# wei-zeng98/piano-a2s

Hardware: AMD Instinct MI355X
Metric: training clips/sec (12 s, 5-bar) (higher is better)
Workload: dtype f32

## Files before the change

### piano_a2s_amd/csrc/a2s_api.hip

```cpp
#define A2S_SWITCHES_IMPL
#include "a2s_internal.h"

thread_local char a2s_err_msg[512] = {0};
long long a2s_launch_counter = 0;

#define ST ((hipStream_t)stream)

extern "C" {

const char* a2s_last_error(void) { return a2s_err_msg; }
int a2s_version(void) { return 1; }
long long a2s_launch_count(void) { return __atomic_load_n(&a2s_launch_counter, __ATOMIC_RELAXED); }

int a2s_gemm_f32(void* stream, int M, int N, int K, float alpha, const float* A, long sAm, long sAk, const float* B, long sBk,
                 long sBn, float beta, float* C, long ldc, const float* bias, int act, int batch, long bsA, long bsB, long bsC,
                 int splitk, float* workspace, size_t workspace_bytes) {
    return a2s_gemm_impl(ST, M, N, K, alpha, A, sAm, sAk, B, sBk, sBn, beta, C, ldc, bias, act, batch, bsA, bsB, bsC, splitk,
                         workspace, workspace_bytes);
}
int a2s_gemm_f32_affine(void* stream, int M, int N, int K, float alpha, const float* A, long sAm, long sAk, const float* B, long sBk,
                        long sBn, float beta, float* C, long ldc, const float* bias, int act, int batch, long bsA, long bsB, long bsC,
                        int splitk, float* workspace, size_t workspace_bytes, const float* a_scale, const float* a_shift, int a_period,
                        const float* b_scale, const float* b_shift, int b_period) {
    return a2s_gemm_affine_impl(ST, M, N, K, alpha, A, sAm, sAk, B, sBk, sBn, beta, C, ldc, bias, act, batch, bsA, bsB, bsC, splitk,
                                workspace, workspace_bytes, a_scale, a_shift, a_period, b_scale, b_shift, b_period,
                                nullptr, nullptr, nullptr, nullptr, nullptr, nullptr, 0, 0, nullptr, nullptr);
}
int a2s_gemm_f32_affine_scaled(void* stream, int M, int N, int K, float alpha, const float* A, long sAm, long sAk, const float* B, long sBk,
                               long sBn, float beta, float* C, long ldc, const float* bias, int act, int batch, long bsA, long bsB, long bsC,
                               int splitk, float* workspace, size_t workspace_bytes, const float* a_scale, const float* a_shift, int a_period,
                               const float* b_scale, const float* b_shift, int b_period, const float* a_absmax, const float* b_absmax) {
    return a2s_gemm_affine_impl(ST, M, N, K, alpha, A, sAm, sAk, B, sBk, sBn, beta, C, ldc, bias, act, batch, bsA, bsB, bsC, splitk,
                                workspace, workspace_bytes, a_scale, a_shift, a_period, b_scale, b_shift, b_period,
                                nullptr, nullptr, nullptr, nullptr, nullptr, nullptr, 0, 1, a_absmax, b_absmax);
}
int a2s_gemm_f32_bnstats_scaled(void* stream, int M, int N, int K, const float* A, long sAm, long sAk, const float* B, long sBk, long sBn, float* C, long ldc,
                                const float* y, const float* mean, const float* invstd, const float* scale, const float* shift, int period, float* partial,
                                const float* a_absmax, const float* b_absmax) {
    return a2s_gemm_affine_impl(ST, M, N, K, 1.f, A, sAm, sAk, B, sBk, sBn, 0.f, C, ldc, nullptr, 0, 1, 0, 0, 0, 1, nullptr, 0,
                                nullptr, nullptr, 0, nullptr, nullptr, 0, y, mean, invstd, scale, shift, partial, period, 1, a_absmax, b_absmax);
}
int a2s_absmax(void* stream, const float* x, long n, float* out) { return a2s_absmax_impl(ST, x, n, out); }
int a2s_linear_dgrad_bnstats(void* stream, int M, int N, int K, const float* dz, long lda, const float* Wt, float* da, long ldc, const float* y,
                             const float* mean, const float* invstd, const float* scale, const float* shift, int period, float* partial,
                             const float* dz_absmax, const float* w_absmax, float* workspace, size_t workspace_bytes, float* da_absmax_out) {
    return a2s_linear_dgrad_bnstats_impl(ST, M, N, K, dz, lda, Wt, 1, K, da, ldc, y, mean, invstd, scale, shift, period, partial, dz_absmax, w_absmax,
                                         workspace, workspace_bytes, da_absmax_out);
}
size_t a2s_linear_dgrad_ws_bytes(int N, int K) { return a2s_linear_dgrad_ws_bytes_impl(N, K); }
int a2s_linear_fwd(void* stream, int M, int N, int K, const float* y, long lda, const float* W, float* z, long ldc, const float* scale, const float* shift,
                   int period, const float* y_absmax, const float* w_absmax, float* workspace, size_t workspace_bytes) {
    return a2s_linear_fwd_impl(ST, M, N, K, y, lda, W, z, ldc, scale, shift, period, y_absmax, w_absmax, workspace, workspace_bytes);
}
int a2s_linear_wgrad(void* stream, int M, int N, int K, const float* dz, long ldz, const float* y, long lda, float* G, long ldg, const float* scale,
                     const float* shift, int period, const float* dz_absmax, const float* y_absmax, float* workspace, size_t workspace_bytes) {
    return a2s_linear_wgrad_impl(ST, M, N, K, dz, ldz, y, lda, G, ldg, scale, shift, period, dz_absmax, y_absmax, workspace, workspace_bytes);
}
size_t a2s_linear_wgrad_ws_bytes(int M, int K) { return a2s_linear_wgrad_ws_bytes_impl(M, K); }
int a2s_linear_wgrad_eligible(int M, int N, int K, int period) { return a2s_linear_wgrad_ok(M, N, K, 256, 4, 4, period, nullptr, nullptr, nullptr) ? 1 : 0; }
int a2s_tallk_wgrad(void* stream, int M, int Np, int K, const float* P, long ldp, const float* A, long lda, float* G, long ldg, int transposed, float* bias,
                    const float* p_absmax, const float* a_absmax, float* workspace, size_t workspace_bytes) {
    return a2s_tallk_wgrad_impl(ST, M, Np, K, P, ldp, A, lda, G, ldg, transposed, bias, p_absmax, a_absmax, workspace, workspace_bytes);
}
size_t a2s_tallk_wgrad_ws_bytes(int M, int Np, int K) { return a2s_tallk_wgrad_ws_bytes_impl(M, Np, K); }
int a2s_tallk_wgrad_eligible(int M, int Np, int K, long ldp, long lda, long ldg, int transposed) {
    return a2s_tallk_wgrad_ok(M, Np, K, ldp, lda, ldg, transposed, nullptr, nullptr, nullptr, nullptr) ? 1 : 0;
}
int a2s_linear_fwd_eligible(int M, int N, int K, int period) { return a2s_linear_fwd_ok(M, N, K, 4, 4, period, nullptr, nullptr, nullptr) ? 1 : 0; }
int a2s_linear_dgrad_blocks(int M) { return a2s_linear_dgrad_blocks_impl(M); }
int a2s_linear_dgrad_eligible(int M, int N, int K, int period) {
    return a2s_linear_dgrad_ok(M, N, K, 4, 1, K, 4, period, nullptr, nullptr, nullptr, nullptr) ? 1 : 0;
}
int a2s_gemm_f32_bnstats(void* stream, int M, int N, int K, const float* A, long sAm, long sAk, const float* B, long sBk, long sBn, float* C, long ldc,
                         const float* y, const float* mean, const float* invstd, const float* scale, const float* shift, int period, float* partial) {
    return a2s_gemm_affine_impl(ST, M, N, K, 1.f, A, sAm, sAk, B, sBk, sBn, 0.f, C, ldc, nullptr, 0, 1, 0, 0, 0, 1, nullptr, 0,
                                nullptr, nullptr, 0, nullptr, nullptr, 0, y, mean, invstd, scale, shift, partial, period, 0, nullptr, nullptr);
}
int a2s_gemm_bnstats_blocks(int M, int period) { return a2s_cdiv(M, 128) * a2s_gemm_bnstats_slots(period); }
size_t a2s_gemm_workspace_bytes(int M, int N, int batch, int splitk) { return a2s_gemm_workspace_bytes_impl(M, N, batch, splitk); }
int a2s_gemm_pick_splitk(int M, int N, int K, int batch) { return a2s_gemm_pick_splitk_impl(M, N, K, batch); }
void a2s_gemm_debug_tile(int cfg) { a2s_gemm_debug_tile_impl(cfg); }
size_t a2s_note_step_workspace_floats(int H, int E) { return a2s_note_step_workspace_floats_impl(H, E); }
int a2s_debug_set(const char* key, int value) {
    if (!key) return A2S_ERR_ARG;
    const int id = a2s_switch_find(key);
    if (id >= 0) { a2s_switch_store(id, value); return A2S_OK; }
    if (!strcmp(key, "attn_deferred_fast")) { a2s_attn_deferred_fast = value ? 1 : 0; return A2S_OK; }
    if (!strcmp(key, "tallk_wgrad")) { a2s_tallk_wgrad_on = value ? 1 : 0; return A2S_OK; }
    if (!strcmp(key, "tallk_wgrad_max_splits")) { a2s_tallk_wgrad_max_splits = value > 0 ? value : 0; return A2S_OK; }
    if (!strcmp(key, "conv_rows_stage")) { a2s_conv_rows_stage = value & 3; return A2S_OK; }
    if (!strcmp(key, "gemm_tile")) { a2s_gemm_debug_tile_impl(value); return A2S_OK; }
    snprintf(a2s_err_msg, sizeof(a2s_err_msg), "a2s_debug_set: unknown key %s", key);
    return A2S_ERR_ARG;
}
int a2s_env_check(void) {
    if (const char* e = a2s_switch_env_error()) A2S_FAIL(A2S_ERR_ARG, "%s: expected a decimal number >= 0", e);
    return A2S_OK;
}

int a2s_persist_abort_latch(void* device_word) { a2s_persist_latch_set(device_word); return A2S_OK; }

int a2s_debug_get(const char* key) {
    if (!key) return -1;
    const int id = a2s_switch_find(key);
    if (id == A2S_SW_attn_pair_fused_rows) return a2s_attn_pair_fused_rows();
    if (id >= 0) return a2s_sw((a2s_switch)id);
    if (!strcmp(key, "attn_pair_launches")) return (int)a2s_attn_pair_launches();
    if (!strcmp(key, "attn_pair_bwd_launches")) return (int)a2s_attn_pair_bwd_launches();
    if (!strcmp(key, "attn_deferred_fast")) return a2s_attn_deferred_fast;
    if (!strcmp(key, "tallk_wgrad")) return a2s_tallk_wgrad_on;
    if (!strcmp(key, "tallk_wgrad_max_splits")) return a2s_tallk_wgrad_max_splits;
    if (!strcmp(key, "tallk_wgrad_launches")) return (int)a2s_tallk_wgrad_launches();
    if (!strcmp(key, "attn_dk_ahead_launches")) return (int)a2s_attn_dk_ahead_launches();
    if (!strcmp(key, "attn_denc_launches")) return (int)a2s_attn_denc_launches();
    if (!strcmp(key, "dec_mid_launches")) return a2s_dec_mid_launches();
    if (!strcmp(key, "dec_cmb_launches")) return a2s_dec_cmb_launches();
    if (!strcmp(key, "dec_persist_launches")) return a2s_dec_persist_launches();
    if (!strcmp(key, "gru_persist_fwd_launches")) return (int)a2s_gru_persist_fwd_launches();
    if (!strcmp(key, "gru_persist_bwd_launches")) return (int)a2s_gru_persist_bwd_launches();
    if (!strcmp(key, "gru_step_fwd_launches")) return (int)a2s_gru_step_fwd_launches();
    if (!strcmp(key, "gru_step_bwd_launches")) return (int)a2s_gru_step_bwd_launches();
    if (!strcmp(key, "edit_distance_launches")) return (int)a2s_edit_distance_launches();
    if (!strcmp(key, "conv_rows16_c20_launches")) return (int)a2s_conv_rows16_c20_launches();
    if (!strcmp(key, "conv_rows_stage")) return a2s_conv_rows_stage;
    if (!strcmp(key, "conv_rows_stage_launches")) return (int)a2s_conv_rows_stage_launches();
    if (!strcmp(key, "device_cus")) return a2s_device_geometry().cus;
    if (!strcmp(key, "device_xccs")) return a2s_device_geometry().xccs;
    return -1;
}

int a2s_conv3x3(void* stream, const float* x, const float* w, float* y, const float* in_scale, const float* in_shift,
                float* stat_partial, int B, int T, int F, int Cin, int Cout, int flip, float* workspace) {
    return a2s_conv3x3_impl(ST, x, w, y, in_scale, in_shift, stat_partial, B, T, F, Cin, Cout, flip, workspace, nullptr, nullptr, nullptr, nullptr, nullptr, nullptr,
                            nullptr, nullptr);
}
int a2s_conv3x3_ranged(void* stream, const float* x, const float* w, float* y, const float* in_scale, const float* in_shift, const float* in_absmax,
                       float* stat_partial, float* out_absmax, int B, int T, int F, int Cin, int Cout, float* workspace) {
    return a2s_conv3x3_impl(ST, x, w, y, in_scale, in_shift, stat_partial, B, T, F, Cin, Cout, 0, workspace, nullptr, nullptr, nullptr, nullptr, nullptr, nullptr,
                            in_absmax, out_absmax);
}
int a2s_conv3x3_dgrad_bnstats(void* stream, const float* dy, const float* w, float* g, const float* yl, const float* yl_mean, const float* yl_invstd,
                              const float* yl_scale, const float* yl_shift, float* stat_partial, int B, int T, int F, int Cin, int Cout,
                              float* workspace) {
    if (!yl) { snprintf(a2s_err_msg, sizeof(a2s_err_msg), "conv3x3_dgrad_bnstats: yl is required"); return A2S_ERR_ARG; }
    return a2s_conv3x3_impl(ST, dy, w, g, nullptr, nullptr, stat_partial, B, T, F, Cin, Cout, 1, workspace, yl, yl_mean, yl_invstd, yl_scale, yl_shift, nullptr, nullptr, nullptr);
}
int a2s_conv3x3_dgrad_bnstats_scaled(void* stream, const float* dy, const float* w, float* g, const float* yl, const float* yl_mean, const float* yl_invstd,
                                     const float* yl_scale, const float* yl_shift, float* stat_partial, int B, int T, int F, int Cin, int Cout,
                                     float* workspace, const float* dy_absmax) {
    if (!yl) { snprintf(a2s_err_msg, sizeof(a2s_err_msg), "conv3x3_dgrad_bnstats_scaled: yl is required"); return A2S_ERR_ARG; }
    return a2s_conv3x3_impl(ST, dy, w, g, nullptr, nullptr, stat_partial, B, T, F, Cin, Cout, 1, workspace, yl, yl_mean, yl_invstd, yl_scale, yl_shift, dy_absmax, nullptr, nullptr);
}
int a2s_conv3x3_dgrad_bnstats_ranged(void* stream, const float* dy, const float* w, float* g, const float* yl, const float* yl_mean, const float* yl_invstd,
                                     const float* yl_scale, const float* yl_shift, float* stat_partial, int B, int T, int F, int Cin, int Cout,
                                     float* workspace, const float* dy_absmax, float* g_absmax_out) {
    if (!yl) { snprintf(a2s_err_msg, sizeof(a2s_err_msg), "conv3x3_dgrad_bnstats_ranged: yl is required"); return A2S_ERR_ARG; }
    return a2s_conv3x3_impl(ST, dy, w, g, nullptr, nullptr, stat_partial, B, T, F, Cin, Cout, 1, workspace, yl, yl_mean, yl_invstd, yl_scale, yl_shift, dy_absmax, nullptr, g_absmax_out);
}
int a2s_bn_bwd_from_partial(void* stream, const float* g, const float* x, const float* mean, const float* invstd, const float* scale, const float* shift,
                            float* dgamma, float* dbeta, float* dx, const float* partial, int nblocks, float* c12, long rows, int C, int F) {
    return a2s_bn_bwd_from_partial_impl(ST, g, x, mean, invstd, scale, shift, dgamma, dbeta, dx, partial, nblocks, c12, rows, C, F, nullptr);
}
int a2s_bn_bwd_from_partial_amax(void* stream, const float* g, const float* x, const float* mean, const float* invstd, const float* scale, const float* shift,
                                 float* dgamma, float* dbeta, float* dx, const float* partial, int nblocks, float* c12, long rows, int C, int F,
                                 float* dx_absmax) {
    return a2s_bn_bwd_from_partial_impl(ST, g, x, mean, invstd, scale, shift, dgamma, dbeta, dx, partial, nblocks, c12, rows, C, F, dx_absmax);
}
size_t a2s_conv3x3_workspace_floats(int Cin) { return a2s_conv3x3_workspace_floats_impl(Cin); }
int a2s_conv3x3_stat_blocks(int B, int T, int F, int Cin) { return a2s_conv3x3_stat_blocks_impl(B, T, F, Cin); }
int a2s_bn_finalize(void* stream, const float* partial, int nblocks, int C, double count, const float* gamma, const float* beta,
                    float* running_mean, float* running_var, long long* nbt, float* mean, float* invstd, float* scale,
                    float* shift, float eps, float momentum, int training) {
    return a2s_bn_finalize_impl(ST, partial, nblocks, C, count, gamma, beta, running_mean, running_var, nbt, mean, invstd, scale,
                                shift, eps, momentum, training);
}
int a2s_bn_relu_apply(void* stream, const float* x, float* y, const float* scale, const float* shift, long n, int C, int F) {
    return a2s_bn_relu_apply_impl(ST, x, y, scale, shift, n, C, F);
}
int a2s_linear_fwd_f64(void* stream, int M, int N, int K, const float* x, const float* W, float* z, const float* scale, const float* shift, int period) {
    return a2s_linear_fwd_f64_impl(ST, M, N, K, x, W, z, scale, shift, period);
}
int a2s_col_stats_split(void* stream, const float* x, float* partial, long rows, int C, int rows_per_block) {
    return a2s_col_stats_split_impl(ST, x, partial, rows, C, rows_per_block);
}
int a2s_col_stats(void* stream, const float* x, float* partial, long rows, int C, int rows_per_block) {
    return a2s_col_stats_impl(ST, x, partial, rows, C, rows_per_block);
}
int a2s_bn1d_relu_dropout(void* stream, const float* x, float* y, const float* scale, const float* shift, const uint8_t* keep_mask,
                          float inv_keep, long n, int C) {
    return a2s_bn1d_relu_dropout_impl(ST, x, y, scale, shift, keep_mask, inv_keep, n, C);
}
int a2s_gru_gates_fwd(void* stream, const float* gi, long ldgi, const float* gh, long ldgh, const float* hprev, long ldhp,
                      float* hout, long ldho, float* hout2, long ldho2, float* save, int R, int H) {
    return a2s_gru_gates_fwd_impl(ST, gi, ldgi, gh, ldgh, hprev, ldhp, hout, ldho, hout2, ldho2, save, R, H);
}
int a2s_gru_seq_fwd(void* stream, const float* gi_all, long gi_bstride, long gi_tstride, const float* w_hh, const float* b_hh,
                    float* out, long out_bstride, long out_tstride, float* hbuf, float* gh, float* save, float* hn, int B, int T,
                    int H, int reverse, float* workspace, size_t workspace_bytes) {
    return a2s_gru_seq_fwd_impl(ST, gi_all, gi_bstride, gi_tstride, w_hh, b_hh, out, out_bstride, out_tstride, hbuf, gh, save, hn,
                                B, T, H, reverse, workspace, workspace_bytes);
}
int a2s_attn_step_fwd(void* stream, const float* keys, const float* enc, const float* q, long ldq, const float* v, float* ctx,
                      long ldctx, float* ctx2, long ldctx2, float* attw, int B, int T, int H, const int* n_done, int n_rows_total, float* workspace) {
    return a2s_attn_step_fwd_impl(ST, keys, enc, q, ldq, v, ctx, ldctx, ctx2, ldctx2, attw, B, T, H, n_done, n_rows_total, workspace, nullptr);
}
int a2s_attn_step_fwd_rows(void* stream, const float* keys, const float* enc, const float* q, long ldq, const float* v, float* ctx,
                           long ldctx, float* ctx2, long ldctx2, float* attw, int R, int T, int H, float* workspace, int n_clips,
                           const int* clip_order, const int* clip_rank, const int* row_until, int n_active, int step) {
// ... 351 lines not shown
```

### piano_a2s_amd/csrc/a2s_internal.h

```cpp
#pragma once
#include "a2s_common.h"
#include "../../include/a2s.h"
#include "a2s_switches.h"

static inline int a2s_attn_pair_fused_rows(void) {
    const int cap = a2s_sw(A2S_SW_dec_fused_max_rows), v = a2s_sw(A2S_SW_attn_pair_fused_rows);
    return v < cap ? v : cap;
}
static inline unsigned a2s_persist_dbg(void) {
    return (a2s_sw(A2S_SW_persist_force_agent) ? PERSIST_DBG_FORCE_AGENT : 0u) | (a2s_sw(A2S_SW_persist_inject_abort) ? PERSIST_DBG_INJECT_ABORT : 0u);
}

int a2s_absmax_impl(hipStream_t st, const float* x, long n, float* out);
size_t a2s_gemm_workspace_bytes_impl(int M, int N, int batch, int splitk);
int a2s_gemm_pick_splitk_impl(int M, int N, int K, int batch);
int a2s_gemm_bnstats_slots(int period);
void a2s_gemm_debug_tile_impl(int cfg);
int a2s_gemm_affine_impl(hipStream_t st, int M, int N, int K, float alpha, const float* A, long sAm, long sAk,
    const float* B, long sBk, long sBn, float beta, float* C, long ldc, const float* bias, int act,
    int batch, long bsA, long bsB, long bsC, int splitk, float* ws, size_t ws_bytes,
    const float* a_scale, const float* a_shift, int a_period, const float* b_scale, const float* b_shift, int b_period,
    const float* ep_y, const float* ep_mean, const float* ep_invstd, const float* ep_scale, const float* ep_shift,
    float* ep_partial, int ep_period, int two_term, const float* a_absmax, const float* b_absmax);
int a2s_gemm_impl(hipStream_t st, int M, int N, int K, float alpha, const float* A, long sAm, long sAk,
    const float* B, long sBk, long sBn, float beta, float* C, long ldc, const float* bias, int act,
    int batch, long bsA, long bsB, long bsC, int splitk, float* ws, size_t ws_bytes);

size_t a2s_linear_dgrad_ws_bytes_impl(int N, int K);
int a2s_linear_dgrad_blocks_impl(int M);
bool a2s_linear_dgrad_ok(int M, int N, int K, long lda, long sBk, long sBn, long ldc, int period, const void* A, const void* B, const void* C, const void* y);
int a2s_linear_dgrad_bnstats_impl(hipStream_t st, int M, int N, int K, const float* A, long lda, const float* Wt, long sBk, long sBn, float* C, long ldc,
    const float* ep_y, const float* mean, const float* invstd, const float* scale, const float* shift, int period,
    float* partial, const float* a_absmax, const float* b_absmax, float* ws, size_t ws_bytes, float* c_absmax_out);
bool a2s_linear_fwd_ok(int M, int N, int K, long lda, long ldc, int period, const void* A, const void* W, const void* C);
int a2s_linear_fwd_impl(hipStream_t st, int M, int N, int K, const float* A, long lda, const float* W, float* C, long ldc, const float* a_scale,
    const float* a_shift, int period, const float* a_absmax, const float* w_absmax, float* ws, size_t ws_bytes);
int a2s_linear_fwd_f64_impl(hipStream_t st, int M, int N, int K, const float* x, const float* W, float* z, const float* scale, const float* shift, int period);
size_t a2s_linear_wgrad_ws_bytes_impl(int M, int K);
bool a2s_linear_wgrad_ok(int M, int N, int K, long ldz, long lda, long ldg, int period, const void* dz, const void* A, const void* G);
int a2s_linear_wgrad_impl(hipStream_t st, int M, int N, int K, const float* dz, long ldz, const float* A, long lda, float* G, long ldg, const float* a_scale,
    const float* a_shift, int period, const float* dz_absmax, const float* a_absmax, float* ws, size_t ws_bytes);
extern int a2s_tallk_wgrad_on;
extern int a2s_tallk_wgrad_max_splits;
long a2s_tallk_wgrad_launches(void);
size_t a2s_tallk_wgrad_ws_bytes_impl(int M, int Np, int K);
bool a2s_tallk_wgrad_ok(int M, int Np, int K, long ldp, long lda, long ldg, int transposed, const void* P, const void* A, const void* G, const void* bias);
int a2s_tallk_wgrad_impl(hipStream_t st, int M, int Np, int K, const float* P, long ldp, const float* A, long lda, float* G, long ldg, int transposed,
    float* bias, const float* p_absmax, const float* a_absmax, float* ws, size_t ws_bytes);

#define CV_TR 4
#define CV_FT 32
#define CV_CK 20
#define C4_TRACE_WGS 8
#define C4_TRACE_STAGES 24
int a2s_act_bound_impl(hipStream_t st, const float* scale, const float* shift, const float* absmax, int C, float* out);
size_t a2s_conv3x3_workspace_floats_impl(int Cin);
int a2s_conv3x3_impl(hipStream_t st, const float* x, const float* w, float* y, const float* in_scale,
    const float* in_shift, float* stat_partial, int B, int T, int F, int Cin, int Cout, int flip, float* ws,
    const float* yl, const float* yl_mean, const float* yl_invstd, const float* yl_scale, const float* yl_shift,
    const float* x_absmax, const float* in_absmax, float* out_absmax);
int a2s_conv3x3_stat_blocks_impl(int B, int T, int F, int Cin);

size_t a2s_conv3x3_wgrad_workspace_bytes_impl(int Cin, int Cout);
int a2s_conv3x3_wgrad_impl(hipStream_t st, const float* dy, const float* x, const float* in_scale, const float* in_shift, float* dW,
    float* ws, size_t ws_bytes, int B, int T, int F, int Cin, int Cout, const float* bn_y, const float* bn_mean,
    const float* bn_invstd, const float* bn_scale, const float* bn_shift, const float* bn_c12, float* dy_out,
    const float* dy_absmax, const float* act_absmax);

int a2s_bn_finalize_impl(hipStream_t st, const float* partial, int nblocks, int C, double count, const float* gamma,
    const float* beta, float* running_mean, float* running_var, long long* nbt, float* mean,
    float* invstd, float* scale, float* shift, float eps, float momentum, int training);
int a2s_bn_relu_apply_impl(hipStream_t st, const float* x, float* y, const float* scale, const float* shift, long n, int C, int F);
int a2s_col_stats_impl(hipStream_t st, const float* x, float* partial, long rows, int C, int rows_per_block);
int a2s_col_stats_split_impl(hipStream_t st, const float* x, float* partial, long rows, int C, int rows_per_block);
int a2s_bn1d_relu_dropout_impl(hipStream_t st, const float* x, float* y, const float* scale, const float* shift,
    const uint8_t* mask, float inv_keep, long n, int C);
int a2s_bn_bwd_impl(hipStream_t st, const float* g, const float* x, const float* mean, const float* invstd, const float* scale,
    const float* shift, const uint8_t* mask, float inv_keep, float* dgamma, float* dbeta, float* dx, float* partial,
    float* c12, long rows, int C, int F, float* dx_absmax);
int a2s_bn_bwd_from_partial_impl(hipStream_t st, const float* g, const float* x, const float* mean, const float* invstd, const float* scale,
    const float* shift, float* dgamma, float* dbeta, float* dx, const float* partial, int nblocks, float* c12,
    long rows, int C, int F, float* dx_absmax);
int a2s_bn_bwd_stats_impl(hipStream_t st, const float* g, const float* x, const float* mean, const float* invstd, const float* scale,
    const float* shift, const uint8_t* mask, float inv_keep, float* partial, float* sums, long rows, int C, int F);
int a2s_bn_bwd_apply_impl(hipStream_t st, const float* g, const float* x, const float* mean, const float* invstd, const float* scale,
    const float* shift, const uint8_t* mask, float inv_keep, const float* sums_local, const float* sums_global,
    double count_global, float* dgamma, float* dbeta, float* dx, float* c12, long rows, int C, int F);
int a2s_bn_bwd_sums_from_partial_impl(hipStream_t st, const float* partial, int nblocks, int C, float* sums);
int a2s_bn_bwd_c12_from_sums_impl(hipStream_t st, const float* sums_local, const float* sums_global, double count_global, float* dgamma, float* dbeta,
    float* c12, int C);
size_t a2s_bn_bwd_partial_floats_impl(long rows, int C, int F);
void a2s_absmax_small_launch(hipStream_t st, const float* w, int n, float* out);

int a2s_channel_absmax_impl(hipStream_t st, const float* x, long rows, int C, int F, float* out);
bool a2s_conv_rows_eligible(int F, int Cin);
int a2s_conv_rows_blocks(int B, int T, int F);
size_t a2s_conv_rows_workspace_floats(int Cin);
long a2s_conv_rows16_c20_launches(void);
extern int a2s_conv_rows_stage;
long a2s_conv_rows_stage_launches(void);
int a2s_conv3x3_rows_impl(hipStream_t st, const float* x, const float* w, float* y, const float* in_scale, const float* in_shift,
    const float* in_absmax, float* stat_partial, float* out_absmax, int B, int T, int F, int Cin, int Cout, int flip,
    float* ws, const float* yl, const float* yl_mean, const float* yl_invstd, const float* yl_scale, const float* yl_shift,
    const float* x_absmax);

bool a2s_wgrad_rows_eligible(int F, int Cin, int Cout);
int a2s_conv3x3_wgrad_rows_bn_impl(hipStream_t st, const float* g, const float* y, const float* mean, const float* invstd, const float* scale,
    const float* shift, const float* c12, const float* g_absmax, int g_absmax_n, const float* y_absmax, float* dz_out,
    float* dz_absmax_out, const float* x, const float* in_scale, const float* in_shift, float* dW, float* ws, size_t ws_bytes,
    int B, int T, int F, int Cin, int Cout, const float* act_absmax);
int a2s_conv3x3_wgrad_rows_impl(hipStream_t st, const float* dy, const float* x, const float* in_scale, const float* in_shift, float* dW, float* ws,
    size_t ws_bytes, int B, int T, int F, int Cin, int Cout, const float* dy_absmax, const float* act_absmax);

struct StepFinArgs {
    const float* logits; long ldl;
    float* probs; long probs_bstride;
    const long long* gt; long gt_bstride;
    const float* emb;
    float* xnext; long ldx;
    const uint8_t* drop; float inv_keep;
    int* argmax_out; long am_bstride;
    int* eos_seen; long long* lengths; int* n_done; int* steps_exec;
    const int* t_base;
    const int* row_until;
    int n_clips;
    int R, V, E, t, teacher_force, eos_id, max_t;
};
struct a2s_grammar_ref { const signed char* next; int n_states; int* row_state; };
struct a2s_metre_ref { const int* dur_ticks; const uint8_t* cls; const uint8_t* fillable; int n_fillable; int* row_metre; };
int a2s_gru_gates_fwd_impl(hipStream_t st, const float* gi, long ldgi, const float* gh, long ldgh, const float* hprev,
    long ldhp, float* hout, long ldho, float* hout2, long ldho2, float* save, int R, int H);
int a2s_gru_bptt_step_impl(hipStream_t st, const float* dgh, const float* w_hh_t, const float* dhz_in, const float* dout, long ld_dout,
    const float* save, const float* hprev, long ld_hprev, float* dgi, long ld_dgi, float* dgh_out, float* dgh2,
    long ld_dgh2, float* dhz_out, int R, int H);
int a2s_skinny_gemm_acc_impl(hipStream_t st, const float* A, long lda, const float* Bt, long ldb, float* Cm, long ldc, int R, int N, int K);
long a2s_gru_step_fwd_launches(void);
long a2s_gru_step_bwd_launches(void);
int a2s_gru_seq_fwd_impl(hipStream_t st, const float* gi_all, long gi_bstride, long gi_tstride, const float* w_hh,
    const float* b_hh, float* out, long out_bstride, long out_tstride, float* hbuf, float* gh,
    float* save, float* hn, int B, int T, int H, int reverse, float* ws, size_t ws_bytes);
int a2s_attn_step_fwd_impl(hipStream_t st, const float* Kmat, const float* enc, const float* q, long ldq, const float* v,
    float* ctx, long ldctx, float* ctx2, long ldctx2, float* attw, int B, int T, int H,
    const int* n_done, int n_rows_total, float* ws, const a2s_attn_rows* rows = nullptr, a2s_attn_deferred* defer = nullptr);
int a2s_log_softmax_rows_impl(hipStream_t st, const float* x, long ldx, float* y, long ldy, int* argmax_out, int R, int V);
int a2s_embed_rows_impl(hipStream_t st, const float* table, const long long* ids64, const int* ids32, long id_stride,
    int const_id, float* out, long ldo, int col0, int R, int E, const uint8_t* drop, float inv_keep);
int a2s_note_decoder_fwd_impl(hipStream_t st, const a2s_note_dec_args& a, int* steps_done);
int a2s_note_decoder_fwd_grammar_impl(hipStream_t st, const a2s_note_dec_args& a, const a2s_grammar_ref& g, int* steps_done);
int a2s_note_decoder_fwd_metre_impl(hipStream_t st, const a2s_note_dec_args& a, const a2s_grammar_ref& g, const a2s_metre_ref* mt, int* steps_done);
int a2s_note_decoder_fwd_pair_impl(hipStream_t su, hipStream_t sl, const a2s_note_dec_args& au, const a2s_note_dec_args& al, const int* pair_order,
    const int* pair_rank, const int* pair_n_active, int* done_u, int* done_l);
int a2s_staff_emb_fwd_impl(hipStream_t st, const float* note_emb, const float* const* w ,
    const long long* ids64, const int* ids32, long id_bstride, const long long* lengths,
    long len_stride, float* out, long ldo, int col0, float* hsave, int R, int maxlen, int E, int S);
int a2s_note_decoder_zero_unwritten(hipStream_t st, const a2s_note_dec_args& a, const char* who );
size_t a2s_attn_workspace_floats_impl(int B, int T, int H, int groups);
size_t a2s_attn_bulk_lds(size_t shm, int n_active, int backward);
long a2s_attn_pair_launches(void);
struct AttnPairStep { const int* clip_order; const int* clip_rank; int n_clips; int n_active; int step; int G; int chunk; };
int a2s_pair_events(const char* who, hipEvent_t** ev_out);
static inline int a2s_record_wait(hipEvent_t ev, hipStream_t from, hipStream_t to, const char* who) {
    hipError_t e = hipEventRecord(ev, from);
    if (e == hipSuccess) e = hipStreamWaitEvent(to, ev, 0);
    if (e != hipSuccess) A2S_FAIL(A2S_ERR_HIP, "%s: event: %s", who, hipGetErrorString(e));
    return A2S_OK;
}

int a2s_log_softmax_bwd_rows_impl(hipStream_t st, const float* g, const float* y, long outer_stride, int inner, float* dx,
    int R, int V, int n_outer, int time_major);
int a2s_gru_gates_bwd_impl(hipStream_t st, const float* dh_a, long lda, const float* dh_b, long ldb, const float* save,
    const float* hprev, long ldhp, float* dgi, long ldgi, float* dgh, long ldgh, float* dgh2, long ldgh2,
    float* dhprev, long lddp, int R, int H);
int a2s_attn_step_bwd_impl(hipStream_t st, const float* Kmat, const float* enc, const float* q, long ldq, const float* v,
    const float* attw, const float* ctx, long ldctx, const float* dctx_a, long ldda, const float* dctx_b,
    long lddb, float* dctx_out, long lddo, float* dq, long lddq, float* ds_out, int B, int T, int H, float* ws,
    const a2s_attn_rows* rows = nullptr);
int a2s_attn_dk_accum_impl(hipStream_t st, const float* Kmat, const float* q_all, const float* ds_all, const float* v,
    float* dK, float* dv_partial, int B, int T, int S, int H, const int* row_until, int groups);
int a2s_attn_denc_accum_impl(hipStream_t st, const float* attw_all, const float* dctx_all, float* dEnc, int B, int T, int S, int H2,
    const int* row_until, int groups);
long a2s_attn_dk_ahead_launches(void);
long a2s_attn_denc_launches(void);
int a2s_col_sum_impl(hipStream_t st, const float* x, long ld, float* out, long rows, int C, float alpha, float beta, float* ws, size_t ws_floats);
// ... 227 lines not shown
```

### piano_a2s_amd/csrc/a2s_linear.hip

```cpp
#include "a2s_internal.h"

#define LIN_BM 128
#define LIN_K 256
#define LIN_RS 288
#define LIN_NTH 512
#define LIN_LDS (2 * 2 * LIN_BM * LIN_RS)

typedef unsigned lu32x4 __attribute__((ext_vector_type(4)));

struct LinDgradArgs {
    const float* A; long lda;
    const unsigned char* planes;
    float* C; long ldc;
    const float* ep_y;
    const float* mean; const float* invstd; const float* scale; const float* shift;
    float* partial;
    const float* a_absmax; const float* b_absmax;
    int M, N, period, channels;
    float* c_absmax_out;
};

__global__ __launch_bounds__(256) void lin_pack_planes_k(const float* __restrict__ W, long ld, int N, int K, const float* __restrict__ absmax,
                                                         unsigned char* __restrict__ out) {
    const long id = (long)blockIdx.x * 256 + threadIdx.x;
    const int kgroups = K >> 3, nks = K >> 5;
    const int n = (int)(id / kgroups), kg = (int)(id % kgroups);
    if (n >= N) return;
    const float ps = ldexpf(1.f, pow2_scale_exp(*absmax, 12));
    const f32x4 v0 = *reinterpret_cast<const f32x4*>(W + (long)n * ld + kg * 8);
    const f32x4 v1 = *reinterpret_cast<const f32x4*>(W + (long)n * ld + kg * 8 + 4);
    float x[8];
#pragma unroll
    for (int i = 0; i < 4; ++i) { x[i] = __builtin_amdgcn_fmed3f(v0[i] * ps, -65000.f, 65000.f); x[4 + i] = __builtin_amdgcn_fmed3f(v1[i] * ps, -65000.f, 65000.f); }
    lu32x4 hi, lo;
#pragma unroll
    for (int i = 0; i < 4; ++i) { unsigned h, l; split2_pair_f16(x[2 * i], x[2 * i + 1], h, l); hi[i] = h; lo[i] = l; }
    const int nt = n >> 4, lr = n & 15, ks = kg >> 2, lk = kg & 3;
    unsigned char* o = out + ((((long)nt * nks + ks) * 2) * 64 + (lk * 16 + lr)) * 16;
    *reinterpret_cast<lu32x4*>(o) = hi;
    *reinterpret_cast<lu32x4*>(o + 64 * 16) = lo;
}

__global__ __launch_bounds__(LIN_NTH) void lin_dgrad_bnstats(LinDgradArgs a) {
    __shared__ __attribute__((aligned(16))) unsigned char lds[LIN_LDS];
    const int tid = threadIdx.x, lane = tid & 63, wave = tid >> 6, lr = lane & 15, lk = lane >> 4;
    const int m0 = blockIdx.x * LIN_BM;
    const int ka = pow2_scale_exp(*a.a_absmax, 12), kb = pow2_scale_exp(*a.b_absmax, 12);
    const float psa = ldexpf(1.f, ka), unscale = ldexpf(1.f, -(ka + kb));

    {
        f32x4 v[16];
#pragma unroll
        for (int i = 0; i < 16; ++i) {
            const int slot = tid + LIN_NTH * i, row = slot >> 6, k = (slot & 63) * 4;
            v[i] = (f32x4){0.f, 0.f, 0.f, 0.f};
            if (m0 + row < a.M) v[i] = *reinterpret_cast<const f32x4*>(a.A + (long)(m0 + row) * a.lda + k);
        }
#pragma unroll
        for (int i = 0; i < 16; ++i) {
            const int slot = tid + LIN_NTH * i, row = slot >> 6, k = (slot & 63) * 4;
            float x[4];
#pragma unroll
            for (int j = 0; j < 4; ++j) x[j] = __builtin_amdgcn_fmed3f(v[i][j] * psa, -65000.f, 65000.f);
            uint2 hi, lo;
            split2_pair_f16(x[0], x[1], hi.x, lo.x);
            split2_pair_f16(x[2], x[3], hi.y, lo.y);
            const int blk = k >> 7, off = (k & 127) * 2;
            *reinterpret_cast<uint2*>(lds + ((blk * 2 + 0) * LIN_BM + row) * LIN_RS + off) = hi;
            *reinterpret_cast<uint2*>(lds + ((blk * 2 + 1) * LIN_BM + row) * LIN_RS + off) = lo;
        }
    }
    __syncthreads();

    const int ntiles = (a.N + 255) >> 8;
    const unsigned lane_off = (unsigned)(lr * a.ldc + lk * 4) * 4u;
    float s1 = 0.f, s2 = 0.f, vmax = 0.f;
    int cur_c = -1;
    auto flush = [&]() {
        if (cur_c < 0) return;
        const float w1 = wave_sum(s1), w2 = wave_sum(s2);
        if (lane == 0) {
            float* p = a.partial + (((long)blockIdx.x * 8 + wave) * a.channels + cur_c) * 2;
            p[0] = w1; p[1] = w2;
// ... 9 lines not shown
    };
    if (wave * 32 < a.N) { load_b(wave * 32, 0, bf[0]); load_b(wave * 32, 1, bf[1]); }
    for (int j = 0; j < ntiles; ++j) {
        const int n0 = j * 256 + wave * 32;
        if (n0 >= a.N) break;
        f32x4 yq[8][2];
        auto load_y = [&](int mt) {
            const int m = m0 + mt * 16 + lr;
#pragma unroll
            for (int nt = 0; nt < 2; ++nt) {
#if defined(LIN_X) && LIN_X >= 1 && LIN_X != 4
                yq[mt][nt] = (f32x4){1.f, 1.f, 1.f, 1.f};
#else
                yq[mt][nt] = (f32x4){0.f, 0.f, 0.f, 0.f};
                if (m < a.M)
                    yq[mt][nt] = *reinterpret_cast<const f32x4*>(reinterpret_cast<const char*>(a.ep_y + (long)(m0 + mt * 16) * a.ldc + n0 + nt * 16) + lane_off);
#endif
            }
        };
#pragma unroll
        for (int mt = 0; mt < 3; ++mt) load_y(mt);
        f32x4 acc[8][2];
#pragma unroll
        for (int mt = 0; mt < 8; ++mt)
#pragma unroll
            for (int nt = 0; nt < 2; ++nt) acc[mt][nt] = (f32x4){0.f, 0.f, 0.f, 0.f};
#pragma unroll
        for (int ks = 0; ks < 8; ++ks) {
#if defined(LIN_X) && LIN_X >= 3
            if (ks + 2 < 8 && a.M < 0) load_b(n0, ks + 2, bf[(ks + 2) % 3]);
#else
            if (ks + 2 < 8) load_b(n0, ks + 2, bf[(ks + 2) % 3]);
#endif
#pragma unroll
            for (int half = 0; half < 2; ++half) {
                lu32x4 af[2][4];
#pragma unroll
                for (int sp = 0; sp < 2; ++sp)
#pragma unroll
                    for (int q = 0; q < 4; ++q)
                        af[sp][q] = *reinterpret_cast<const lu32x4*>(lds + (((ks >> 2) * 2 + sp) * LIN_BM + (half * 4 + q) * 16 + lr) * LIN_RS + (ks & 3) * 64 + lk * 16);
#define LIN_PRODUCT(SA, SB)                                                                                                   \
                _Pragma("unroll") for (int nt = 0; nt < 2; ++nt)                                                              \
                    _Pragma("unroll") for (int q = 0; q < 4; ++q)                                                             \
                        acc[half * 4 + q][nt] = __builtin_amdgcn_mfma_f32_16x16x32_f16(__builtin_bit_cast(f16x8, bf[ks % 3][nt][SB]), \
                                                                                       __builtin_bit_cast(f16x8, af[SA][q]), acc[half * 4 + q][nt], 0, 0, 0);
                LIN_PRODUCT(1, 0) LIN_PRODUCT(0, 1) LIN_PRODUCT(0, 0)
#undef LIN_PRODUCT
            }
        }
        if (n0 + 256 < a.N) { load_b(n0 + 256, 0, bf[0]); load_b(n0 + 256, 1, bf[1]); }
#pragma unroll
        for (int mt = 3; mt < 8; ++mt) load_y(mt);
        const int c = n0 / a.period;
        if (c != cur_c) { flush(); s1 = 0.f; s2 = 0.f; cur_c = c; }
        const float mean = a.mean[c], invstd = a.invstd[c], sc = a.scale[c], sh = a.shift[c];
#pragma unroll
        for (int mt = 0; mt < 8; ++mt) {
            const int m = m0 + mt * 16 + lr;
            if (m >= a.M) continue;
#pragma unroll
            for (int nt = 0; nt < 2; ++nt) {
                f32x4 v = acc[mt][nt];
#pragma unroll
                for (int r = 0; r < 4; ++r) { v[r] *= unscale; vmax = fmaxf(vmax, fabsf(v[r])); }
#if defined(LIN_X) && LIN_X >= 2
                if (v[0] == 123.456f)
#endif
                *reinterpret_cast<f32x4*>(reinterpret_cast<char*>(a.C + (long)(m0 + mt * 16) * a.ldc + n0 + nt * 16) + lane_off) = v;
#pragma unroll
                for (int r = 0; r < 4; ++r) {
                    const float gm = (fmaf(yq[mt][nt][r], sc, sh) > 0.f) ? v[r] : 0.f;
                    s1 += gm; s2 = fmaf(gm * (yq[mt][nt][r] - mean), invstd, s2);
                }
            }
        }
    }
    flush();
    if (a.c_absmax_out) {
        const float m = wave_max(vmax);
        if (lane == 0 && m > 0.f) atomicMax(reinterpret_cast<unsigned*>(a.c_absmax_out), __float_as_uint(m));
    }
}

size_t a2s_linear_dgrad_ws_bytes_impl(int N, int K) { return (K > 0 && K % 32 == 0 && N > 0) ? (size_t)N * K * 2 * 2 : 0; }
int a2s_linear_dgrad_blocks_impl(int M) { return M > 0 ? ((M + LIN_BM - 1) / LIN_BM) * 8 : 0; }

bool a2s_linear_dgrad_ok(int M, int N, int K, long lda, long sBk, long sBn, long ldc, int period, const void* A, const void* B, const void* C, const void* y) {
    return K == LIN_K && M >= LIN_BM && N >= 256 && N % 32 == 0 && period > 0 && period % 32 == 0 && N % period == 0 && N / period <= 4096 && sBk == 1 && sBn == K &&
           lda % 4 == 0 && ldc % 4 == 0 && (((uintptr_t)A | (uintptr_t)B | (uintptr_t)C | (uintptr_t)y) % 16 == 0);
}

int a2s_linear_dgrad_bnstats_impl(hipStream_t st, int M, int N, int K, const float* A, long lda, const float* Wt, long sBk, long sBn, float* C, long ldc,
                                  const float* ep_y, const float* mean, const float* invstd, const float* scale, const float* shift, int period,
                                  float* partial, const float* a_absmax, const float* b_absmax, float* ws, size_t ws_bytes, float* c_absmax_out) {
    A2S_REQUIRE(A && Wt && C && ep_y && mean && invstd && scale && shift && partial && a_absmax && b_absmax && ws, "linear_dgrad_bnstats: null argument");
    A2S_REQUIRE(a2s_linear_dgrad_ok(M, N, K, lda, sBk, sBn, ldc, period, A, Wt, C, ep_y),
                "linear_dgrad_bnstats: needs K = 256, M >= 128, N >= 256, N %% 32 == 0, period %% 32 == 0, a k-contiguous weight (N x K) and 16-byte aligned rows");
    A2S_REQUIRE(((uintptr_t)ws % 16 == 0) && ws_bytes >= a2s_linear_dgrad_ws_bytes_impl(N, K), "linear_dgrad_bnstats: workspace too small (%zu bytes needed)",
                a2s_linear_dgrad_ws_bytes_impl(N, K));
    const int channels = N / period, nblk = a2s_linear_dgrad_blocks_impl(M);
    hipError_t e = hipMemsetAsync(partial, 0, sizeof(float) * 2 * (size_t)nblk * channels, st);
    if (e != hipSuccess) A2S_FAIL(A2S_ERR_HIP, "linear_dgrad_bnstats memset: %s", hipGetErrorString(e));
    unsigned char* planes = reinterpret_cast<unsigned char*>(ws);
    hipLaunchKernelGGL(lin_pack_planes_k, dim3((unsigned)(((long)N * (K / 8) + 255) / 256)), dim3(256), 0, st, Wt, (long)K, N, K, b_absmax, planes);
    A2S_CHECK_LAUNCH("lin_pack_planes_k");
    LinDgradArgs a{A, lda, planes, C, ldc, ep_y, mean, invstd, scale, shift, partial, a_absmax, b_absmax, M, N, period, channels, c_absmax_out};
    hipLaunchKernelGGL(lin_dgrad_bnstats, dim3((M + LIN_BM - 1) / LIN_BM), dim3(LIN_NTH), 0, st, a);
    A2S_CHECK_LAUNCH("lin_dgrad_bnstats");
    return A2S_OK;
}

#define LF_RS 160
#define LF_STAGE (2 * LIN_BM * LF_RS)
#define LF_NS 3

struct LinFwdArgs {
    const float* A; long lda;
    const unsigned char* planes;
    float* C; long ldc;
    const float* a_scale; const float* a_shift;
    const float* a_absmax; const float* b_absmax;
    int M, K, period;
};

__global__ __launch_bounds__(LIN_NTH) void lin_fwd_roles(LinFwdArgs a) {
    __shared__ __attribute__((aligned(16))) unsigned char lds[LF_NS * LF_STAGE];
    const int tid = threadIdx.x, lane = tid & 63, lr = lane & 15, lk = lane >> 4;
    const int wave = __builtin_amdgcn_readfirstlane(tid >> 6);
    const int m0 = blockIdx.x * LIN_BM;
    const int ka = a.a_absmax ? pow2_scale_exp(*a.a_absmax, 12) : 0, kb = pow2_scale_exp(*a.b_absmax, 12);
    const float psa = ldexpf(1.f, ka), unscale = ldexpf(1.f, -(ka + kb));
    const int nks = a.K >> 5, nblk = a.K >> 6, kpc = a.period >> 5;
    const bool affine = a.a_scale != nullptr;
    if (wave >= 4) {
        const int st_ = tid - 256;
        const int sk = (st_ & 15) * 4;
        const bool second = sk >= 32;
        f32x4 ar[2][8];
        auto issue_a = [&](int blk, f32x4 (&r)[8]) {
#pragma unroll
            for (int i = 0; i < 8; ++i) {
                const int row = (st_ + 256 * i) >> 4;
                r[i] = (f32x4){0.f, 0.f, 0.f, 0.f};
                if (m0 + row < a.M && blk < nblk) r[i] = __builtin_nontemporal_load(reinterpret_cast<const f32x4*>(a.A + (long)(m0 + row) * a.lda + (long)blk * 64 + sk));
            }
        };
        auto commit_a = [&](int blk, const f32x4 (&r)[8]) {
            if (blk >= nblk) return;
            const int c0 = (2 * blk) / kpc, c1 = (2 * blk + 1) / kpc;
            const float sc = affine ? (second ? a.a_scale[c1] : a.a_scale[c0]) * psa : psa, sh = affine ? (second ? a.a_shift[c1] : a.a_shift[c0]) * psa : 0.f;
            const float floor_ = affine ? 0.f : -INFINITY;
            unsigned char* st = lds + (blk % LF_NS) * LF_STAGE;
#pragma unroll
            for (int i = 0; i < 8; ++i) {
                const int row = (st_ + 256 * i) >> 4;
                float x[4];
#pragma unroll
                for (int j = 0; j < 4; ++j) x[j] = __builtin_amdgcn_fmed3f(fmaxf(fmaf(r[i][j], sc, sh), floor_), -65000.f, 65000.f);
                uint2 hi, lo;
                split2_pair_f16(x[0], x[1], hi.x, lo.x);
                split2_pair_f16(x[2], x[3], hi.y, lo.y);
                *reinterpret_cast<uint2*>(st + (0 * LIN_BM + row) * LF_RS + sk * 2) = hi;
                *reinterpret_cast<uint2*>(st + (1 * LIN_BM + row) * LF_RS + sk * 2) = lo;
            }
        };
        issue_a(0, ar[0]);
        commit_a(0, ar[0]);
        issue_a(1, ar[1]); issue_a(2, ar[0]);
#pragma unroll 1
        for (int b0 = 0; b0 < nblk; b0 += 2) {
            __syncthreads();
            commit_a(b0 + 1, ar[1]); issue_a(b0 + 3, ar[1]);
            if (b0 + 1 < nblk) {
                __syncthreads();
                commit_a(b0 + 2, ar[0]); issue_a(b0 + 4, ar[0]);
            }
        }
        return;
    }
    lu32x4 bf[2][4][2];
    auto load_b = [&](int ks, lu32x4 (&dst)[4][2]) {
        if (ks >= nks) return;
#pragma unroll
        for (int nt = 0; nt < 4; ++nt)
#pragma unroll
            for (int sp = 0; sp < 2; ++sp)
                dst[nt][sp] = *reinterpret_cast<const lu32x4*>(a.planes + (((long)(wave * 4 + nt) * nks + ks) * 2 + sp) * 1024 + (unsigned)lane * 16u);
    };
    f32x4 acc[8][4];
#pragma unroll
// ... 432 lines not shown
```

Baseline: 641.2.

## Add software-pipelined linear dgrad kernel with BN-stats epilogue prefetching

Adds a new variant of the linear dgrad + batch-norm-stats kernel. It triple-buffers the packed weight-plane fragments two k-steps ahead, prefetches the next tile's weight planes and epilogue y values during the current epilogue, and specialises the loop on full versus partial row blocks. The aim is to hide global load latency behind the MFMA work and the epilogue. The new kernel is on by default and can be switched off through a debug key. In exchange it holds more registers for the buffered fragments and y values, which may lower occupancy.

```diff
diff --git a/piano_a2s_amd/csrc/a2s_api.hip b/piano_a2s_amd/csrc/a2s_api.hip
--- a/piano_a2s_amd/csrc/a2s_api.hip
+++ b/piano_a2s_amd/csrc/a2s_api.hip
@@ -89,6 +89,7 @@
     if (!strcmp(key, "tallk_wgrad")) { a2s_tallk_wgrad_on = value ? 1 : 0; return A2S_OK; }
     if (!strcmp(key, "tallk_wgrad_max_splits")) { a2s_tallk_wgrad_max_splits = value > 0 ? value : 0; return A2S_OK; }
     if (!strcmp(key, "conv_rows_stage")) { a2s_conv_rows_stage = value & 3; return A2S_OK; }
+    if (!strcmp(key, "lin_dgrad_pipe")) { a2s_lin_dgrad_pipe = value ? 1 : 0; return A2S_OK; }
     if (!strcmp(key, "gemm_tile")) { a2s_gemm_debug_tile_impl(value); return A2S_OK; }
     snprintf(a2s_err_msg, sizeof(a2s_err_msg), "a2s_debug_set: unknown key %s", key);
     return A2S_ERR_ARG;
@@ -124,6 +125,8 @@
     if (!strcmp(key, "conv_rows16_c20_launches")) return (int)a2s_conv_rows16_c20_launches();
     if (!strcmp(key, "conv_rows_stage")) return a2s_conv_rows_stage;
     if (!strcmp(key, "conv_rows_stage_launches")) return (int)a2s_conv_rows_stage_launches();
+    if (!strcmp(key, "lin_dgrad_pipe")) return a2s_lin_dgrad_pipe;
+    if (!strcmp(key, "lin_dgrad_pipe_launches")) return (int)a2s_lin_dgrad_pipe_launches();
     if (!strcmp(key, "device_cus")) return a2s_device_geometry().cus;
     if (!strcmp(key, "device_xccs")) return a2s_device_geometry().xccs;
     return -1;
diff --git a/piano_a2s_amd/csrc/a2s_internal.h b/piano_a2s_amd/csrc/a2s_internal.h
--- a/piano_a2s_amd/csrc/a2s_internal.h
+++ b/piano_a2s_amd/csrc/a2s_internal.h
@@ -99,6 +99,8 @@
 long a2s_conv_rows16_c20_launches(void);
 extern int a2s_conv_rows_stage;
 long a2s_conv_rows_stage_launches(void);
+extern int a2s_lin_dgrad_pipe;
+long a2s_lin_dgrad_pipe_launches(void);
 int a2s_conv3x3_rows_impl(hipStream_t st, const float* x, const float* w, float* y, const float* in_scale, const float* in_shift,
     const float* in_absmax, float* stat_partial, float* out_absmax, int B, int T, int F, int Cin, int Cout, int flip,
     float* ws, const float* yl, const float* yl_mean, const float* yl_invstd, const float* yl_scale, const float* yl_shift,
diff --git a/piano_a2s_amd/csrc/a2s_linear.hip b/piano_a2s_amd/csrc/a2s_linear.hip
--- a/piano_a2s_amd/csrc/a2s_linear.hip
+++ b/piano_a2s_amd/csrc/a2s_linear.hip
@@ -1,4 +1,5 @@
 #include "a2s_internal.h"
+#include <type_traits>
 
 #define LIN_BM 128
 #define LIN_K 256
@@ -174,6 +175,163 @@
         if (lane == 0 && m > 0.f) atomicMax(reinterpret_cast<unsigned*>(a.c_absmax_out), __float_as_uint(m));
     }
 }
+
+__global__ __launch_bounds__(LIN_NTH) void lin_dgrad_bnstats_pipe(LinDgradArgs a) {
+    __shared__ __attribute__((aligned(16))) unsigned char lds[LIN_LDS];
+    const int tid = threadIdx.x, lane = tid & 63, lr = lane & 15, lk = lane >> 4;
+    const int wave = __builtin_amdgcn_readfirstlane(tid >> 6);
+    const int m0 = blockIdx.x * LIN_BM;
+    const bool full = m0 + LIN_BM <= a.M;
+    const int ka = pow2_scale_exp(*a.a_absmax, 12), kb = pow2_scale_exp(*a.b_absmax, 12);
+    const float psa = ldexpf(1.f, ka), unscale = ldexpf(1.f, -(ka + kb));
+
+    {
+        f32x4 v[16];
+#pragma unroll
+        for (int i = 0; i < 16; ++i) {
+            const int slot = tid + LIN_NTH * i, row = slot >> 6, k = (slot & 63) * 4;
+            v[i] = (f32x4){0.f, 0.f, 0.f, 0.f};
+            if (m0 + row < a.M) v[i] = *reinterpret_cast<const f32x4*>(a.A + (long)(m0 + row) * a.lda + k);
+        }
+#pragma unroll
+        for (int i = 0; i < 16; ++i) {
+            const int slot = tid + LIN_NTH * i, row = slot >> 6, k = (slot & 63) * 4;
+            float x[4];
+#pragma unroll
+            for (int j = 0; j < 4; ++j) x[j] = __builtin_amdgcn_fmed3f(v[i][j] * psa, -65000.f, 65000.f);
+            uint2 hi, lo;
+            split2_pair_f16(x[0], x[1], hi.x, lo.x);
+            split2_pair_f16(x[2], x[3], hi.y, lo.y);
+            const int blk = k >> 7, off = (k & 127) * 2;
+            *reinterpret_cast<uint2*>(lds + ((blk * 2 + 0) * LIN_BM + row) * LIN_RS + off) = hi;
+            *reinterpret_cast<uint2*>(lds + ((blk * 2 + 1) * LIN_BM + row) * LIN_RS + off) = lo;
+        }
+    }
+    unsigned lane_off = (unsigned)(lr * a.ldc + lk * 4) * 4u;
+    unsigned abase[4];
+#pragma unroll
+    for (int b = 0; b < 4; ++b) {
+        abase[b] = (unsigned)((b * LIN_BM + lr) * LIN_RS + lk * 16);
+        asm volatile("" : "+v"(abase[b]));
+    }
+    float s1 = 0.f, s2 = 0.f, vmax = 0.f;
+    int cur_c = -1;
+    auto flush = [&]() {
+        if (cur_c < 0) return;
+        const float w1 = wave_sum(s1), w2 = wave_sum(s2);
+        if (lane == 0) {
+            float* p = a.partial + (((long)blockIdx.x * 8 + wave) * a.channels + cur_c) * 2;
+            p[0] = w1; p[1] = w2;
+        }
+    };
+    lu32x4 bf[3][2][2];
+    auto load_b = [&](int n0, int ks, lu32x4 (&dst)[2][2]) {
+        const unsigned char* bp = a.planes + (long)(n0 >> 4) * 8 * 2 * 64 * 16;
+#pragma unroll
+        for (int nt = 0; nt < 2; ++nt)
+#pragma unroll
+            for (int sp = 0; sp < 2; ++sp) dst[nt][sp] = *reinterpret_cast<const lu32x4*>(bp + ((long)(nt * 8 + ks) * 2 + sp) * 1024 + (unsigned)lane * 16u);
+    };
+    f32x4 yq[8][2];
+    auto load_y = [&](int n0, int mt) {
+#pragma unroll
+        for (int nt = 0; nt < 2; ++nt) {
+#if defined(LIN_X) && LIN_X >= 1 && LIN_X != 4
+            yq[mt][nt] = (f32x4){1.f, 1.f, 1.f, 1.f};
+#else
+            yq[mt][nt] = *reinterpret_cast<const f32x4*>(reinterpret_cast<const char*>(a.ep_y + (long)(m0 + mt * 16) * a.ldc + n0 + nt * 16) + lane_off);
+#endif
+        }
+    };
+#pragma unroll
+    for (int mt = 0; mt < 8; ++mt) { yq[mt][0] = (f32x4){0.f, 0.f, 0.f, 0.f}; yq[mt][1] = (f32x4){0.f, 0.f, 0.f, 0.f}; }
+
+    auto tile = [&](int n0, auto full_, auto next_) __attribute__((always_inline)) {
+        constexpr bool FULL = decltype(full_)::value, NEXT = decltype(next_)::value;
+        asm volatile("" : "+v"(lane_off));
+        const int c = n0 / a.period;
+        const float mean = a.mean[c], invstd = a.invstd[c], sc = a.scale[c], sh = a.shift[c];
+        f32x4 acc[8][2];
+#pragma unroll
+        for (int mt = 0; mt < 8; ++mt)
+#pragma unroll
+            for (int nt = 0; nt < 2; ++nt) acc[mt][nt] = (f32x4){0.f, 0.f, 0.f, 0.f};
+#pragma unroll
+        for (int ks = 0; ks < 8; ++ks) {
+#if defined(LIN_X) && LIN_X >= 3
+            if (ks + 2 < 8 && a.M < 0) load_b(n0, ks + 2, bf[(ks + 2) % 3]);
+#else
+            if (ks + 2 < 8) load_b(n0, ks + 2, bf[(ks + 2) % 3]);
+#endif
+#ifndef LIN_PIPE_NOKFENCE
+            __builtin_amdgcn_sched_barrier(0);
+#endif
+#pragma unroll
+            for (int half = 0; half < 2; ++half) {
+                lu32x4 af[2][4];
+#pragma unroll
+                for (int sp = 0; sp < 2; ++sp)
+#pragma unroll
+                    for (int q = 0; q < 4; ++q)
+                        af[sp][q] = *reinterpret_cast<const lu32x4*>(lds + abase[(ks >> 2) * 2 + sp] + (half * 4 + q) * 16 * LIN_RS + (ks & 3) * 64);
+#define LIN_PRODUCT(SA, SB)                                                                                                   \
+                _Pragma("unroll") for (int nt = 0; nt < 2; ++nt)                                                              \
+                    _Pragma("unroll") for (int q = 0; q < 4; ++q)                                                             \
+                        acc[half * 4 + q][nt] = __builtin_amdgcn_mfma_f32_16x16x32_f16(__builtin_bit_cast(f16x8, bf[ks % 3][nt][SB]), \
+                                                                                       __builtin_bit_cast(f16x8, af[SA][q]), acc[half * 4 + q][nt], 0, 0, 0);
+                LIN_PRODUCT(1, 0) LIN_PRODUCT(0, 1) LIN_PRODUCT(0, 0)
+#undef LIN_PRODUCT
+            }
+        }
+        __builtin_amdgcn_sched_barrier(0);
+        if (NEXT) { load_b(n0 + 256, 0, bf[0]); load_b(n0 + 256, 1, bf[1]); }
+        if (c != cur_c) { flush(); s1 = 0.f; s2 = 0.f; cur_c = c; }
+#pragma unroll
+        for (int mt = 0; mt < 8; ++mt) {
+            __builtin_amdgcn_sched_barrier(0);
+            if (!FULL && m0 + mt * 16 + lr >= a.M) continue;
+#pragma unroll
+            for (int nt = 0; nt < 2; ++nt) {
+                f32x4 v = acc[mt][nt];
+#pragma unroll
+                for (int r = 0; r < 4; ++r) { v[r] *= unscale; vmax = fmaxf(vmax, fabsf(v[r])); }
+#if defined(LIN_X) && LIN_X >= 2
+                if (v[0] == 123.456f)
+#endif
+                *reinterpret_cast<f32x4*>(reinterpret_cast<char*>(a.C + (long)(m0 + mt * 16) * a.ldc + n0 + nt * 16) + lane_off) = v;
+#pragma unroll
+                for (int r = 0; r < 4; ++r) {
+                    const float gm = (fmaf(yq[mt][nt][r], sc, sh) > 0.f) ? v[r] : 0.f;
+                    s1 += gm; s2 = fmaf(gm * (yq[mt][nt][r] - mean), invstd, s2);
+                }
+            }
+            if (NEXT) load_y(n0 + 256, mt);
+        }
+        __builtin_amdgcn_sched_barrier(0);
+    };
+    auto run = [&](auto full_) __attribute__((always_inline)) {
+        constexpr bool FULL = decltype(full_)::value;
+        load_b(wave * 32, 0, bf[0]); load_b(wave * 32, 1, bf[1]);
+#pragma unroll
+        for (int mt = 0; mt < 8; ++mt)
+            if (FULL || m0 + mt * 16 + lr < a.M) load_y(wave * 32, mt);
+        __syncthreads();
+        int n0 = wave * 32;
+        for (; n0 + 256 < a.N; n0 += 256) tile(n0, full_, std::true_type{});
+        tile(n0, full_, std::false_type{});
+        flush();
+        if (a.c_absmax_out) {
+            const float m = wave_max(vmax);
+            if (lane == 0 && m > 0.f) atomicMax(reinterpret_cast<unsigned*>(a.c_absmax_out), __float_as_uint(m));
+        }
+    };
+    if (full) run(std::true_type{});
+    else run(std::false_type{});
+}
+
+int a2s_lin_dgrad_pipe = 1;
+static long g_lin_dgrad_pipe_launches = 0;
+long a2s_lin_dgrad_pipe_launches(void) { return (long)__atomic_load_n(&g_lin_dgrad_pipe_launches, __ATOMIC_RELAXED); }
 
 size_t a2s_linear_dgrad_ws_bytes_impl(int N, int K) { return (K > 0 && K % 32 == 0 && N > 0) ? (size_t)N * K * 2 * 2 : 0; }
 int a2s_linear_dgrad_blocks_impl(int M) { return M > 0 ? ((M + LIN_BM - 1) / LIN_BM) * 8 : 0; }
@@ -198,7 +356,12 @@
     hipLaunchKernelGGL(lin_pack_planes_k, dim3((unsigned)(((long)N * (K / 8) + 255) / 256)), dim3(256), 0, st, Wt, (long)K, N, K, b_absmax, planes);
     A2S_CHECK_LAUNCH("lin_pack_planes_k");
     LinDgradArgs a{A, lda, planes, C, ldc, ep_y, mean, invstd, scale, shift, partial, a_absmax, b_absmax, M, N, period, channels, c_absmax_out};
-    hipLaunchKernelGGL(lin_dgrad_bnstats, dim3((M + LIN_BM - 1) / LIN_BM), dim3(LIN_NTH), 0, st, a);
+    if (a2s_lin_dgrad_pipe) {
+        hipLaunchKernelGGL(lin_dgrad_bnstats_pipe, dim3((M + LIN_BM - 1) / LIN_BM), dim3(LIN_NTH), 0, st, a);
+        __atomic_fetch_add(&g_lin_dgrad_pipe_launches, 1, __ATOMIC_RELAXED);
+    } else {
+        hipLaunchKernelGGL(lin_dgrad_bnstats, dim3((M + LIN_BM - 1) / LIN_BM), dim3(LIN_NTH), 0, st, a);
+    }
     A2S_CHECK_LAUNCH("lin_dgrad_bnstats");
     return A2S_OK;
 }
```

Result: no change. 643.1, median of 5 (+0.3%).
